# stevenczwu/SAMBLE

Measured on NVIDIA B200. Metric: clouds/sec SAMBLE seg fwd (N=2048), higher is better.
Workload: dtype f32

## Files before the change

samble_b200/csrc/edgeconv_tc.cu:

```cuda
#include "common.cuh"
#include "tc_common.cuh"

namespace samble {

constexpr int kEtThreads = 416;
constexpr int kEtStages = 4;

__device__ __forceinline__ unsigned f2ord(float f) {
  const unsigned u = __float_as_uint(f);
  return (u & 0x80000000u) ? ~u : (u | 0x80000000u);
}
__device__ __forceinline__ float ord2f(unsigned u) { return __uint_as_float((u & 0x80000000u) ? (u & 0x7fffffffu) : ~u); }

template <class I, int C2>
__global__ void __launch_bounds__(kEtThreads, 1)
    edge_mlp_tc_kernel(const float* __restrict__ pr, long long ld_pr, const I* __restrict__ idx, const float* __restrict__ w2,
                       const float* __restrict__ b2, int B, int N, int K, int C1, float* __restrict__ out, long long out_ld, int dbg) {
  extern __shared__ uint8_t smem_raw[];
  uint8_t* base = tc::smem_align1024(smem_raw);
  const int nkb = C1 / 32;
  constexpr int kWBlock = C2 * 128;
  uint8_t* sWh = base;
  uint8_t* sWl = sWh + (size_t)nkb * kWBlock;
  uint8_t* sH = sWl + (size_t)nkb * kWBlock;
  uint64_t* bars = reinterpret_cast<uint64_t*>(sH + (size_t)kEtStages * 32768);
  uint64_t* full = bars;
  uint64_t* empty = bars + kEtStages;
  uint64_t* tfull = empty + kEtStages;
  uint64_t* tempty = tfull + 2;
  uint32_t* tmem_slot = reinterpret_cast<uint32_t*>(tempty + 2);

  const int tid = threadIdx.x, warp = tid >> 5, lane = tid & 31;
  const int tiles_per_cloud = (N + 3) / 4;
  const int total = B * tiles_per_cloud;

  for (int p = tid; p < nkb * C2 * 8; p += kEtThreads) {
    const int kb = p / (C2 * 8), row = (p / 8) % C2, ch = p & 7;
    const float4 v = __ldg(reinterpret_cast<const float4*>(w2 + (size_t)row * C1 + kb * 32 + ch * 4));
    float4 lo;
    lo.x = v.x - __uint_as_float(__float_as_uint(v.x) & 0xffffe000u);
    lo.y = v.y - __uint_as_float(__float_as_uint(v.y) & 0xffffe000u);
    lo.z = v.z - __uint_as_float(__float_as_uint(v.z) & 0xffffe000u);
    lo.w = v.w - __uint_as_float(__float_as_uint(v.w) & 0xffffe000u);
    const uint32_t off = (uint32_t)kb * kWBlock + tc::sw128_offset(row, ch);
    *reinterpret_cast<float4*>(sWh + off) = v;
    *reinterpret_cast<float4*>(sWl + off) = lo;
  }
  tc::fence_proxy_async();
  if (tid == 0) {
    for (int s = 0; s < kEtStages; ++s) {
      tc::mbar_init(&full[s], 4);
      tc::mbar_init(&empty[s], 1);
    }
    for (int i = 0; i < 2; ++i) {
      tc::mbar_init(&tfull[i], 1);
      tc::mbar_init(&tempty[i], 4);
    }
    tc::mbar_init_fence();
  }
  if (warp == 0) tc::tmem_alloc(tmem_slot, 2 * C2);
  tc::tc_fence_before();
  __syncthreads();
  tc::tc_fence_after();
  const uint32_t tmem = *tmem_slot;

  if (warp >= 5) {
    const int grp = (warp - 5) >> 2, lw = (warp - 5) & 3;
    const int sub = lane & 7, rsel = lane >> 3;
    const int ntl = (total - (int)blockIdx.x + (int)gridDim.x - 1) / (int)gridDim.x;
    const int G = ntl * nkb;
    float4 pv, rv[8];
    auto fetch = [&](int g) {
      const int tile = blockIdx.x + (g / nkb) * gridDim.x, kb = g % nkb;
      const int b = tile / tiles_per_cloud, n = (tile % tiles_per_cloud) * 4 + lw;
      const bool ok = n < N;
      const long long prow = (long long)b * N + (ok ? n : 0);
      const int j = ok ? ld_idx(idx, prow * K + min(lane, K - 1)) : 0;
      pv = ok ? __ldg(reinterpret_cast<const float4*>(pr + prow * ld_pr + kb * 32) + sub) : make_float4(0.f, 0.f, 0.f, 0.f);
      const float* rbase = pr + (long long)b * N * ld_pr + C1 + kb * 32;
#pragma unroll
      for (int t = 0; t < 8; ++t) {
        const int jr = __shfl_sync(kFull, j, t * 4 + rsel);
        rv[t] = ok ? __ldg(reinterpret_cast<const float4*>(rbase + (long long)jr * ld_pr) + sub) : make_float4(0.f, 0.f, 0.f, 0.f);
      }
    };
    if (grp < G && !(dbg & 1)) fetch(grp);
    for (int g = grp; g < G; g += 2) {
      const int s = g % kEtStages;
      tc::mbar_wait(&empty[s], ((g / kEtStages) & 1) ^ 1);
      uint8_t* hh = sH + (size_t)s * 32768;
      uint8_t* hl = hh + 16384;
      if (!(dbg & 8))
#pragma unroll
      for (int t = 0; t < 8; ++t) {
        float4 h;
        h.x = pv.x + rv[t].x, h.y = pv.y + rv[t].y, h.z = pv.z + rv[t].z, h.w = pv.w + rv[t].w;
        h.x = h.x > 0.f ? h.x : 0.2f * h.x;
        h.y = h.y > 0.f ? h.y : 0.2f * h.y;
        h.z = h.z > 0.f ? h.z : 0.2f * h.z;
        h.w = h.w > 0.f ? h.w : 0.2f * h.w;
        float4 lo;
        lo.x = h.x - __uint_as_float(__float_as_uint(h.x) & 0xffffe000u);
        lo.y = h.y - __uint_as_float(__float_as_uint(h.y) & 0xffffe000u);
        lo.z = h.z - __uint_as_float(__float_as_uint(h.z) & 0xffffe000u);
        lo.w = h.w - __uint_as_float(__float_as_uint(h.w) & 0xffffe000u);
        const uint32_t off = tc::sw128_offset(lw * 32 + t * 4 + rsel, sub);
        *reinterpret_cast<float4*>(hh + off) = h;
        *reinterpret_cast<float4*>(hl + off) = lo;
      }
      if (g + 2 < G && !(dbg & 1)) fetch(g + 2);
      tc::fence_proxy_async();
      __syncwarp();
      if (lane == 0) tc::mbar_arrive(&full[s]);
    }
  } else if (warp == 4) {
    if (tc::elect_one()) {
      const uint32_t idesc = tc::instr_desc(2, 128, C2);
      int g = 0, it = 0;
      for (int tile = blockIdx.x; tile < total; tile += gridDim.x, ++it) {
        const int set = it & 1;
        tc::mbar_wait(&tempty[set], ((it >> 1) & 1) ^ 1);
        tc::tc_fence_after();
        for (int kb = 0; kb < nkb; ++kb, ++g) {
          const int s = g % kEtStages;
          tc::mbar_wait(&full[s], (g / kEtStages) & 1);
          tc::tc_fence_after();
          const uint32_t st = tc::smem_u32(sH + (size_t)s * 32768);
          const uint64_t hh = tc::smem_desc_sw128(st), hl = tc::smem_desc_sw128(st + 16384);
          const uint64_t wh = tc::smem_desc_sw128(tc::smem_u32(sWh + (size_t)kb * kWBlock));
          const uint64_t wl = tc::smem_desc_sw128(tc::smem_u32(sWl + (size_t)kb * kWBlock));
          const uint32_t acc = tmem + set * C2;
          if (!(dbg & 2))
#pragma unroll
          for (int k8 = 0; k8 < 4; ++k8) {
            tc::mma_tf32(acc, hh + 2 * k8, wh + 2 * k8, idesc, (kb | k8) != 0);
            tc::mma_tf32(acc, hl + 2 * k8, wh + 2 * k8, idesc, 1);
            tc::mma_tf32(acc, hh + 2 * k8, wl + 2 * k8, idesc, 1);
          }
          tc::mma_commit(&empty[s]);
        }
        tc::mma_commit(&tfull[set]);
      }
    }
    __syncwarp();
  } else {
    int it = 0;
    for (int tile = blockIdx.x; tile < total; tile += gridDim.x, ++it) {
      const int set = it & 1;
      const int b = tile / tiles_per_cloud, n = (tile % tiles_per_cloud) * 4 + warp;
      tc::mbar_wait(&tfull[set], (it >> 1) & 1);
      tc::tc_fence_after();
      const uint32_t taddr = tmem + ((uint32_t)(warp * 32) << 16) + set * C2;
      if (!(dbg & 4))
#pragma unroll 1
      for (int c0 = 0; c0 < C2; c0 += 32) {
        float v[32];
        tc::tmem_ld32(taddr + c0, v);
#pragma unroll
        for (int w = 16; w >= 1; w >>= 1) {
          const bool upper = (lane & w) != 0;
#pragma unroll
          for (int i = 0; i < w; ++i) {
            const float keep = upper ? v[i + w] : v[i], send = upper ? v[i] : v[i + w];
            v[i] = fmaxf(keep, __shfl_xor_sync(kFull, send, w));
          }
        }
        const float mine = v[0];
        if (n < N) {
          const int c = c0 + lane;
          const float y = mine + __ldg(b2 + c);
          out[out_ld ? ((long long)b * N + n) * out_ld + c : ((long long)b * C2 + c) * N + n] = y > 0.f ? y : 0.2f * y;
        }
      }
      tc::tc_fence_before();
      __syncwarp();
      if (lane == 0) tc::mbar_arrive(&tempty[set]);
    }
  }
  tc::tc_fence_before();
  __syncthreads();
  if (warp == 0) tc::tmem_dealloc(tmem, 2 * C2);
}

int g_edge_debug = 0;

template <class I, int C2>
static int launch_edge_tc(const float* pr, long long ld_pr, const I* idx, const float* w2, const float* b2, int B, int N,
                          int K, int C1, float* out, long long out_ld, cudaStream_t st) {
  const int nkb = C1 / 32;
  size_t smem = (size_t)2 * nkb * C2 * 128 + (size_t)kEtStages * 32768 + 1024 + 256;
  auto kern = edge_mlp_tc_kernel<I, C2>;
  if (cudaFuncSetAttribute(kern, cudaFuncAttributeMaxDynamicSharedMemorySize, (int)smem) != cudaSuccess)
    return check_launch("edge_mlp_tc smem attribute");
  const long long total = (long long)B * ((N + 3) / 4);
  const int grid = (int)(total < 148 ? total : 148);
  SAMBLE_PRE(st);
  kern<<<grid, kEtThreads, smem, st>>>(pr, ld_pr, idx, w2, b2, B, N, K, C1, out, out_ld, g_edge_debug);
  SAMBLE_LAUNCHED("edge_mlp_tc_kernel");
  return SAMBLE_OK;
}

bool edge_tc_eligible(int K, int C1, int C2) {
  if (!(K <= 32 && C1 % 32 == 0 && C1 <= 128 && (C2 == 64 || C2 == 128))) return false;
  return (size_t)2 * (C1 / 32) * C2 * 128 + (size_t)kEtStages * 32768 + 1280 <= 225 * 1024;
}

template <class I>
int edge_mlp_tc(const float* pr, long long ld_pr, const I* idx, const float* w2, const float* b2, int B, int N, int K, int C1,
                int C2, float* out, long long out_ld, cudaStream_t st) {
  if (C2 == 64) return launch_edge_tc<I, 64>(pr, ld_pr, idx, w2, b2, B, N, K, C1, out, out_ld, st);
  return launch_edge_tc<I, 128>(pr, ld_pr, idx, w2, b2, B, N, K, C1, out, out_ld, st);
}
template int edge_mlp_tc<int>(const float*, long long, const int*, const float*, const float*, int, int, int, int, int, float*, long long, cudaStream_t);
template int edge_mlp_tc<long long>(const float*, long long, const long long*, const float*, const float*, int, int, int, int, int, float*, long long, cudaStream_t);

}

extern "C" void samble_set_edge_debug(int bits) { samble::g_edge_debug = bits; }
```

Before: 4977.

## Transpose edge-conv MMA so weights form M and eight points' neighbors form N

Swaps the tcgen05 TF32 MMA operands so output channels lie along TMEM lanes and 8 points × 32 neighbors lie along columns. The max over neighbors then becomes a per-thread register reduction instead of a 31-step shuffle butterfly. Tiles grow from 4 to 8 points with 8 producer warps per group, and stages are 64 KB with the stage count sized from the remaining shared memory. All 512 TMEM columns are allocated, and the next gather now starts after the barrier arrive. For C2=64 the M=128 MMA reads past the weight block into unused rows, and a kernel holding all of TMEM limits co-residency.

```diff
diff --git a/samble_b200/csrc/edgeconv_tc.cu b/samble_b200/csrc/edgeconv_tc.cu
--- a/samble_b200/csrc/edgeconv_tc.cu
+++ b/samble_b200/csrc/edgeconv_tc.cu
@@ -3,19 +3,19 @@
 
 namespace samble {
 
-constexpr int kEtThreads = 416;
-constexpr int kEtStages = 4;
-
-__device__ __forceinline__ unsigned f2ord(float f) {
-  const unsigned u = __float_as_uint(f);
-  return (u & 0x80000000u) ? ~u : (u | 0x80000000u);
-}
-__device__ __forceinline__ float ord2f(unsigned u) { return __uint_as_float((u & 0x80000000u) ? (u & 0x7fffffffu) : ~u); }
+constexpr int kEtThreads = 672;
+constexpr int kEtPoints = 8;
+constexpr int kEtStage = 65536;
+constexpr int kEtSmemMax = 227 * 1024;
+
+constexpr size_t edge_w_bytes(int C1, int C2) { return (size_t)2 * (C1 / 32) * C2 * 128; }
+static int edge_stages(int C1, int C2) { return (int)((kEtSmemMax - edge_w_bytes(C1, C2) - 1280) / kEtStage); }
 
 template <class I, int C2>
 __global__ void __launch_bounds__(kEtThreads, 1)
     edge_mlp_tc_kernel(const float* __restrict__ pr, long long ld_pr, const I* __restrict__ idx, const float* __restrict__ w2,
-                       const float* __restrict__ b2, int B, int N, int K, int C1, float* __restrict__ out, long long out_ld, int dbg) {
+                       const float* __restrict__ b2, int B, int N, int K, int C1, float* __restrict__ out, long long out_ld,
+                       int nst, int dbg) {
   extern __shared__ uint8_t smem_raw[];
   uint8_t* base = tc::smem_align1024(smem_raw);
   const int nkb = C1 / 32;
@@ -23,15 +23,15 @@
   uint8_t* sWh = base;
   uint8_t* sWl = sWh + (size_t)nkb * kWBlock;
   uint8_t* sH = sWl + (size_t)nkb * kWBlock;
-  uint64_t* bars = reinterpret_cast<uint64_t*>(sH + (size_t)kEtStages * 32768);
+  uint64_t* bars = reinterpret_cast<uint64_t*>(sH + (size_t)nst * kEtStage);
   uint64_t* full = bars;
-  uint64_t* empty = bars + kEtStages;
-  uint64_t* tfull = empty + kEtStages;
+  uint64_t* empty = bars + nst;
+  uint64_t* tfull = empty + nst;
   uint64_t* tempty = tfull + 2;
   uint32_t* tmem_slot = reinterpret_cast<uint32_t*>(tempty + 2);
 
   const int tid = threadIdx.x, warp = tid >> 5, lane = tid & 31;
-  const int tiles_per_cloud = (N + 3) / 4;
+  const int tiles_per_cloud = (N + kEtPoints - 1) / kEtPoints;
   const int total = B * tiles_per_cloud;
 
   for (int p = tid; p < nkb * C2 * 8; p += kEtThreads) {
@@ -48,31 +48,31 @@
   }
   tc::fence_proxy_async();
   if (tid == 0) {
-    for (int s = 0; s < kEtStages; ++s) {
-      tc::mbar_init(&full[s], 4);
+    for (int s = 0; s < nst; ++s) {
+      tc::mbar_init(&full[s], kEtPoints);
       tc::mbar_init(&empty[s], 1);
     }
     for (int i = 0; i < 2; ++i) {
       tc::mbar_init(&tfull[i], 1);
-      tc::mbar_init(&tempty[i], 4);
+      tc::mbar_init(&tempty[i], C2 / 32);
     }
     tc::mbar_init_fence();
   }
-  if (warp == 0) tc::tmem_alloc(tmem_slot, 2 * C2);
+  if (warp == 0) tc::tmem_alloc(tmem_slot, 512);
   tc::tc_fence_before();
   __syncthreads();
   tc::tc_fence_after();
   const uint32_t tmem = *tmem_slot;
 
   if (warp >= 5) {
-    const int grp = (warp - 5) >> 2, lw = (warp - 5) & 3;
+    const int grp = (warp - 5) >> 3, lw = (warp - 5) & 7;
     const int sub = lane & 7, rsel = lane >> 3;
     const int ntl = (total - (int)blockIdx.x + (int)gridDim.x - 1) / (int)gridDim.x;
     const int G = ntl * nkb;
     float4 pv, rv[8];
     auto fetch = [&](int g) {
       const int tile = blockIdx.x + (g / nkb) * gridDim.x, kb = g % nkb;
-      const int b = tile / tiles_per_cloud, n = (tile % tiles_per_cloud) * 4 + lw;
+      const int b = tile / tiles_per_cloud, n = (tile % tiles_per_cloud) * kEtPoints + lw;
       const bool ok = n < N;
       const long long prow = (long long)b * N + (ok ? n : 0);
       const int j = ok ? ld_idx(idx, prow * K + min(lane, K - 1)) : 0;
@@ -86,10 +86,10 @@
     };
     if (grp < G && !(dbg & 1)) fetch(grp);
     for (int g = grp; g < G; g += 2) {
-      const int s = g % kEtStages;
-      tc::mbar_wait(&empty[s], ((g / kEtStages) & 1) ^ 1);
-      uint8_t* hh = sH + (size_t)s * 32768;
-      uint8_t* hl = hh + 16384;
+      const int s = g % nst;
+      tc::mbar_wait(&empty[s], ((g / nst) & 1) ^ 1);
+      uint8_t* hh = sH + (size_t)s * kEtStage;
+      uint8_t* hl = hh + kEtStage / 2;
       if (!(dbg & 8))
 #pragma unroll
       for (int t = 0; t < 8; ++t) {
@@ -108,34 +108,34 @@
         *reinterpret_cast<float4*>(hh + off) = h;
         *reinterpret_cast<float4*>(hl + off) = lo;
       }
-      if (g + 2 < G && !(dbg & 1)) fetch(g + 2);
       tc::fence_proxy_async();
       __syncwarp();
       if (lane == 0) tc::mbar_arrive(&full[s]);
+      if (g + 2 < G && !(dbg & 1)) fetch(g + 2);
     }
   } else if (warp == 4) {
     if (tc::elect_one()) {
-      const uint32_t idesc = tc::instr_desc(2, 128, C2);
+      const uint32_t idesc = tc::instr_desc(2, 128, kEtPoints * 32);
       int g = 0, it = 0;
       for (int tile = blockIdx.x; tile < total; tile += gridDim.x, ++it) {
         const int set = it & 1;
         tc::mbar_wait(&tempty[set], ((it >> 1) & 1) ^ 1);
         tc::tc_fence_after();
         for (int kb = 0; kb < nkb; ++kb, ++g) {
-          const int s = g % kEtStages;
-          tc::mbar_wait(&full[s], (g / kEtStages) & 1);
+          const int s = g % nst;
+          tc::mbar_wait(&full[s], (g / nst) & 1);
           tc::tc_fence_after();
-          const uint32_t st = tc::smem_u32(sH + (size_t)s * 32768);
-          const uint64_t hh = tc::smem_desc_sw128(st), hl = tc::smem_desc_sw128(st + 16384);
+          const uint32_t st = tc::smem_u32(sH + (size_t)s * kEtStage);
+          const uint64_t hh = tc::smem_desc_sw128(st), hl = tc::smem_desc_sw128(st + kEtStage / 2);
           const uint64_t wh = tc::smem_desc_sw128(tc::smem_u32(sWh + (size_t)kb * kWBlock));
           const uint64_t wl = tc::smem_desc_sw128(tc::smem_u32(sWl + (size_t)kb * kWBlock));
-          const uint32_t acc = tmem + set * C2;
+          const uint32_t acc = tmem + set * (kEtPoints * 32);
           if (!(dbg & 2))
 #pragma unroll
           for (int k8 = 0; k8 < 4; ++k8) {
-            tc::mma_tf32(acc, hh + 2 * k8, wh + 2 * k8, idesc, (kb | k8) != 0);
-            tc::mma_tf32(acc, hl + 2 * k8, wh + 2 * k8, idesc, 1);
-            tc::mma_tf32(acc, hh + 2 * k8, wl + 2 * k8, idesc, 1);
+            tc::mma_tf32(acc, wh + 2 * k8, hh + 2 * k8, idesc, (kb | k8) != 0);
+            tc::mma_tf32(acc, wh + 2 * k8, hl + 2 * k8, idesc, 1);
+            tc::mma_tf32(acc, wl + 2 * k8, hh + 2 * k8, idesc, 1);
           }
           tc::mma_commit(&empty[s]);
         }
@@ -143,32 +143,27 @@
       }
     }
     __syncwarp();
-  } else {
+  } else if (warp * 32 < C2) {
+    const int c = warp * 32 + lane;
+    const float bias = __ldg(b2 + c);
     int it = 0;
     for (int tile = blockIdx.x; tile < total; tile += gridDim.x, ++it) {
       const int set = it & 1;
-      const int b = tile / tiles_per_cloud, n = (tile % tiles_per_cloud) * 4 + warp;
+      const int b = tile / tiles_per_cloud, n0 = (tile % tiles_per_cloud) * kEtPoints;
       tc::mbar_wait(&tfull[set], (it >> 1) & 1);
       tc::tc_fence_after();
-      const uint32_t taddr = tmem + ((uint32_t)(warp * 32) << 16) + set * C2;
+      const uint32_t taddr = tmem + ((uint32_t)(warp * 32) << 16) + set * (kEtPoints * 32);
       if (!(dbg & 4))
 #pragma unroll 1
-      for (int c0 = 0; c0 < C2; c0 += 32) {
+      for (int p = 0; p < kEtPoints; ++p) {
         float v[32];
-        tc::tmem_ld32(taddr + c0, v);
-#pragma unroll
-        for (int w = 16; w >= 1; w >>= 1) {
-          const bool upper = (lane & w) != 0;
-#pragma unroll
-          for (int i = 0; i < w; ++i) {
-            const float keep = upper ? v[i + w] : v[i], send = upper ? v[i] : v[i + w];
-            v[i] = fmaxf(keep, __shfl_xor_sync(kFull, send, w));
-          }
-        }
-        const float mine = v[0];
+        tc::tmem_ld32(taddr + p * 32, v);
+        float m = v[0];
+#pragma unroll
+        for (int i = 1; i < 32; ++i) m = fmaxf(m, v[i]);
+        const int n = n0 + p;
         if (n < N) {
-          const int c = c0 + lane;
-          const float y = mine + __ldg(b2 + c);
+          const float y = m + bias;
           out[out_ld ? ((long long)b * N + n) * out_ld + c : ((long long)b * C2 + c) * N + n] = y > 0.f ? y : 0.2f * y;
         }
       }
@@ -179,7 +174,7 @@
   }
   tc::tc_fence_before();
   __syncthreads();
-  if (warp == 0) tc::tmem_dealloc(tmem, 2 * C2);
+  if (warp == 0) tc::tmem_dealloc(tmem, 512);
 }
 
 int g_edge_debug = 0;
@@ -187,22 +182,21 @@
 template <class I, int C2>
 static int launch_edge_tc(const float* pr, long long ld_pr, const I* idx, const float* w2, const float* b2, int B, int N,
                           int K, int C1, float* out, long long out_ld, cudaStream_t st) {
-  const int nkb = C1 / 32;
-  size_t smem = (size_t)2 * nkb * C2 * 128 + (size_t)kEtStages * 32768 + 1024 + 256;
+  const int nst = edge_stages(C1, C2);
+  const size_t smem = edge_w_bytes(C1, C2) + (size_t)nst * kEtStage + 1024 + 256;
   auto kern = edge_mlp_tc_kernel<I, C2>;
   if (cudaFuncSetAttribute(kern, cudaFuncAttributeMaxDynamicSharedMemorySize, (int)smem) != cudaSuccess)
     return check_launch("edge_mlp_tc smem attribute");
-  const long long total = (long long)B * ((N + 3) / 4);
+  const long long total = (long long)B * ((N + kEtPoints - 1) / kEtPoints);
   const int grid = (int)(total < 148 ? total : 148);
   SAMBLE_PRE(st);
-  kern<<<grid, kEtThreads, smem, st>>>(pr, ld_pr, idx, w2, b2, B, N, K, C1, out, out_ld, g_edge_debug);
+  kern<<<grid, kEtThreads, smem, st>>>(pr, ld_pr, idx, w2, b2, B, N, K, C1, out, out_ld, nst, g_edge_debug);
   SAMBLE_LAUNCHED("edge_mlp_tc_kernel");
   return SAMBLE_OK;
 }
 
 bool edge_tc_eligible(int K, int C1, int C2) {
-  if (!(K <= 32 && C1 % 32 == 0 && C1 <= 128 && (C2 == 64 || C2 == 128))) return false;
-  return (size_t)2 * (C1 / 32) * C2 * 128 + (size_t)kEtStages * 32768 + 1280 <= 225 * 1024;
+  return K <= 32 && C1 % 32 == 0 && C1 <= 128 && (C2 == 64 || C2 == 128) && edge_w_bytes(C1, C2) <= 65536;
 }
 
 template <class I>
```

After: 5087 (median of 6 runs). 2.2% higher.
